# manish-pra/sampling-gpmpc

Measured on AMD Instinct MI355X. Metric: sampled trajectory-steps/sec (Ns*H per wall second), higher is better.
Workload: dtype f64; 1 GPU; BASELINE configs[1]: params_pendulum1D_samples, sequential re-conditioned rollout (mode R, value+gradient labels T=3), Ns=1024 per GPU, H=30; Ns_per_gpu=1024, H=30, Ns_total=1024, device=AMD Radeon Graphics (gfx950:sramecc+:xnack-), cus=256

## Files before the change

### sampling_gpmpc_amd/csrc/rollout_one.hip

```cpp
#include "gpmpc_host.hpp"
#include "rollout_plan.hpp"

#include <type_traits>
#include <utility>

namespace gpmpc {

#include "rollout_one_gen.inc"
#include "rollout_one_steps_gen.inc"

__device__ long long g_one_phase_cycles[16];
__device__ double g_one_dbg[64 * 64];

#ifdef GPMPC_PHASE_TIMERS
#define OPH_DECL long long oph_[10] = {0, 0, 0, 0, 0, 0, 0, 0, 0, 0}; long long opht_ = __builtin_readcyclecounter()
#define OPH(i) do { const long long n_ = __builtin_readcyclecounter(); oph_[i] += n_ - opht_; opht_ = n_; } while (0)
#define OPH_T(i) OPH(i)
#define OPH_STORE do { if (blockIdx.x == 0 && threadIdx.x == 0) { for (int i_ = 0; i_ < 8; ++i_) g_one_phase_cycles[i_] = oph_[i_]; g_one_phase_cycles[10] = oph_[8]; g_one_phase_cycles[11] = oph_[9]; } } while (0)
#elif defined(GPMPC_ONE_PHASE_MARKS)
#define OPH_DECL
#define OPH(i) asm volatile("; one_phase_end " #i)
#define OPH_T(i)
#define OPH_STORE
#else
// ... 207 lines not shown
    if (rk < 0) return OV_OLD;
    if (rk > ri) return OV_ZERO;
    return ri == 0 ? OV_C00 : (ri == 1 ? OV_C10 + rk : OV_C20 + rk);
}
constexpr int one_new_inv(int i) { return (i >= 0 && i < 3) ? OV_CI0 + i : OV_KEEP; }
template <int I0, int BT>
struct OnePatReach {
    static constexpr int at(int kq, int bm, int jq) {
        return (bm == BT && jq < I0 - 1 && kq >= I0) ? one_new_entry(4 + jq - I0, kq - I0) : OV_KEEP;
    }
};
template <int LO>
struct OnePatDiag {
    static constexpr int at(int kq, int bm, int jq) {
        const int ri = 4 * bm + jq - LO;
        return (ri >= 0 && ri < 3) ? one_new_entry(ri, 4 * bm + kq - LO) : OV_KEEP;
    }
};
template <int LO>
struct OnePatInvRow {
    static constexpr int at(int kq, int bm, int) { return one_new_inv(4 * bm + kq - LO); }
};
template <int LO>
struct OnePatInvCol {
    static constexpr int at(int, int bm, int jq) { return one_new_inv(4 * bm + jq - LO); }
};

struct OneCholPair {
    double d0[2], y0[2], r0[2];
};
#ifdef GPMPC_ONE_NO_REST_FENCES
#define GPMPC_ONE_FENCE()
#else
#define GPMPC_ONE_FENCE() __builtin_amdgcn_sched_barrier(0)
#endif
#define GPMPC_ONE_LVL(stmt, third)                              \
    _Pragma("unroll") for (int m_ = 0; m_ < 2; ++m_) { stmt; }  \
    third;                                                      \
    GPMPC_ONE_FENCE()
__device__ __forceinline__ void one_chol_pivot1(double a00, double b00, OneCholPair& p) {
    double h[2], t[2], e[2];
    p.d0[0] = a00, p.d0[1] = b00;
    __builtin_amdgcn_sched_barrier(0);
    GPMPC_ROW2L(p.y0[m_] = __builtin_amdgcn_rsq(p.d0[m_]); h[m_] = 0.5 * p.d0[m_]);
    GPMPC_ROW2L(t[m_] = h[m_] * p.y0[m_]);
    GPMPC_ROW2L(e[m_] = fma(-t[m_], p.y0[m_], 0.5));
    GPMPC_ROW2L(p.y0[m_] = fma(p.y0[m_], e[m_], p.y0[m_]));
    GPMPC_ROW2L(p.r0[m_] = p.d0[m_] * p.y0[m_]);
}
__device__ __forceinline__ void one_chol_rest(const double (&A)[3][3], const double (&B)[3][3], const OneCholPair& p, double x,
                                              const OneExpConsts& k, double (&LA)[3][3], double (&LB)[3][3], double (&invA)[3],
                                              double (&invB)[3], bool& okA, bool& okB, double& ex) {
    double s10[2] = {A[1][0], B[1][0]}, s20[2] = {A[2][0], B[2][0]}, s21[2] = {A[2][1], B[2][1]};
    double s11[2] = {A[1][1], B[1][1]}, s22[2] = {A[2][2], B[2][2]};
    double d1[2], d2[2], y1[2], y2[2], h[2], t[2], e[2], l10[2], l20[2], l21[2], n21[2], p2[2], r1[2], r2[2];
    double n, r, rr, a0, a1, a2, a4;
    int ni;
    GPMPC_ONE_FENCE();
    GPMPC_ONE_LVL(l10[m_] = s10[m_] * p.y0[m_]; l20[m_] = s20[m_] * p.y0[m_], n = x * k.log2e);
    GPMPC_ONE_LVL(d1[m_] = fma(-l10[m_], l10[m_], s11[m_]); n21[m_] = fma(-l20[m_], l10[m_], s21[m_]), n = rint(n));
    GPMPC_ONE_LVL(y1[m_] = __builtin_amdgcn_rsq(d1[m_]); h[m_] = 0.5 * d1[m_]; p2[m_] = fma(-l20[m_], l20[m_], s22[m_]),
                  r = fma(n, k.nln2h, x));
    GPMPC_ONE_LVL(t[m_] = h[m_] * y1[m_], r = fma(n, k.nln2l, r); ni = (int)n);
    GPMPC_ONE_LVL(e[m_] = fma(-t[m_], y1[m_], 0.5), rr = r * r; a0 = 1.0 + r; a1 = fma(k.c3, r, k.c2));
    GPMPC_ONE_LVL(y1[m_] = fma(y1[m_], e[m_], y1[m_]), a0 = fma(a1, rr, a0); a4 = fma(k.c9, r, k.c8); a1 = fma(k.c11, r, k.c10));
    GPMPC_ONE_LVL(l21[m_] = n21[m_] * y1[m_]; r1[m_] = d1[m_] * y1[m_], a4 = fma(a1, rr, a4); a2 = fma(k.c5, r, k.c4));
    GPMPC_ONE_LVL(d2[m_] = fma(-l21[m_], l21[m_], p2[m_]), a1 = fma(k.c7, r, k.c6));
    GPMPC_ONE_LVL(y2[m_] = __builtin_amdgcn_rsq(d2[m_]); h[m_] = 0.5 * d2[m_], a2 = fma(a1, rr, a2); rr = rr * rr);
    GPMPC_ONE_LVL(t[m_] = h[m_] * y2[m_], a2 = fma(a4, rr, a2));
    GPMPC_ONE_LVL(e[m_] = fma(-t[m_], y2[m_], 0.5), a0 = fma(a2, rr, a0));
    GPMPC_ONE_LVL(y2[m_] = fma(y2[m_], e[m_], y2[m_]), ex = ldexp(a0, ni));
    GPMPC_ONE_LVL(r2[m_] = d2[m_] * y2[m_], (void)0);
    asm volatile("" ::"v"(p.r0[0]), "v"(r1[0]), "v"(r2[0]), "v"(p.r0[1]), "v"(r1[1]), "v"(r2[1]));
    okA = (p.d0[0] > 0.0) && (d1[0] > 0.0) && (d2[0] > 0.0);
    okB = (p.d0[1] > 0.0) && (d1[1] > 0.0) && (d2[1] > 0.0);
    LA[0][0] = p.r0[0], LA[1][0] = l10[0], LA[2][0] = l20[0], LA[1][1] = r1[0], LA[2][1] = l21[0], LA[2][2] = r2[0];
    LB[0][0] = p.r0[1], LB[1][0] = l10[1], LB[2][0] = l20[1], LB[1][1] = r1[1], LB[2][1] = l21[1], LB[2][2] = r2[1];
    LA[0][1] = LA[0][2] = LA[1][2] = 0.0;
    LB[0][1] = LB[0][2] = LB[1][2] = 0.0;
    invA[0] = p.y0[0], invA[1] = y1[0], invA[2] = y2[0];
    invB[0] = p.y0[1], invB[1] = y1[1], invB[2] = y2[1];
}

typedef const __attribute__((address_space(4))) RolloutArgs* OneArgsPtr;
typedef __attribute__((address_space(3))) double* OneLdsRow;
__device__ __forceinline__ OneArgsPtr one_cold_args(OneArgsPtr p) {
    asm volatile("" : "+s"(p));
    return p;
}
__device__ __forceinline__ long one_cold_sample(int s) {
    asm volatile("" : "+s"(s));
    return s;
}

__device__ __forceinline__ bool one_wanted(double* p) {
    asm volatile("" : "+s"(p));
    return p != nullptr;
}
struct OneLds {
    static constexpr int VR = 0;
    static constexpr int HS = ((4 * kOneNKT * kOneRS + 1) & ~1);
    static constexpr int TOTAL = HS + 96 * kOneRS;
};

constexpr int one_epoch_of(int t) { return (kOneNKT + ((3 * t) >> 2)) >> 2; }
template <int N0, int ENV, bool LEAN, bool STEPS>
__device__ __forceinline__ void rollout_one_body(const RolloutArgs& a) {
    static_assert(ENV == GPMPC_ENV_PENDULUM1D && N0 == 4, "instantiated for the pendulum1D 4 x 9 grid");
    constexpr int D = 2, T = 3, N1 = 9, NR = N0 * N1, NX = 2;
    constexpr int NKT = kOneNKT;
    constexpr int KFIRST = NKT >> 2, KLAST = (NKT + kOneNTR - 1) >> 2;
    static_assert(4 * NKT == NR && N0 + N1 <= 16, "panel map generated for N_r = 36");
    extern __shared__ __attribute__((aligned(16))) double smem[];
#ifdef GPMPC_PHASE_TIMERS
    const long long opk0_ = __builtin_readcyclecounter();
#endif

    const GpParams& gp = a.gp;
    const OneArgsPtr ak0 = (OneArgsPtr)__builtin_amdgcn_kernarg_segment_ptr();
    const int s32 = blockIdx.x;
    const int lane = threadIdx.x;
    const int kq = lane >> 4, bm = (lane >> 2) & 3, jq = lane & 3;
    const long s = blockIdx.x;
    const int H = a.H;
    double* VRb = smem + OneLds::VR;
    double* HSb = smem + OneLds::HS;

    const double il0 = gp.inv_l2[0][0], il1 = gp.inv_l2[0][1], os = gp.os[0];
    const int lr = (lane < NR) ? lane : 0, ga = lr / N1, gc = lr - ga * N1;
    double qa[N0], qb[N1];
#pragma unroll
    for (int j = 0; j < N0; ++j) qa[j] = plan_grid_Qa(a.plan, gp, 0)[j * N0 + ga];
#pragma unroll
    for (int j = 0; j < N1; ++j) qb[j] = plan_grid_Qb(a.plan, gp, 0)[j * N1 + gc];
    double dsc_ld = plan_grid_dsc(a.plan, gp, 0)[lr], w_ld = plan_grid_w(a.plan, gp, 0)[lr];
    const bool g_ax0 = lane < N0;
    const int g_pt = g_ax0 ? lane * N1 : ((lane < N0 + N1) ? lane - N0 : 0);
    const bool g_axis = lane < N0 + N1, g_sel0 = g_ax0 || !g_axis;
    double g_x = a.X_r[g_pt * D + (g_ax0 ? 0 : 1)];
    const double il0_lane = g_axis ? (g_ax0 ? il0 : il1) : il0, il1_lane = g_axis ? 0.0 : il1;
    const int bp_addr = (lane & 15) << 2;
    constexpr int kPt0 = N0 + N1;
    const int jpt = lane - kPt0;
    const double Inat = (kq == jq) ? 1.0 : 0.0;
    const double MK[4] = {(bm == 0) ? 1.0 : 0.0, (bm == 1) ? 1.0 : 0.0, (bm == 2) ? 1.0 : 0.0, (bm == 3) ? 1.0 : 0.0};
    const int vr_rd = (4 * bm + kq) * kOneRS + jq;
    const int hs_rd = (4 * (bm - NKT) + kq) * kOneRS + jq;
    unsigned hs_wr = (unsigned)(size_t)(OneLdsRow)(HSb + 3 * jpt * kOneRS), vr_wr = (unsigned)(size_t)(OneLdsRow)(VRb + lane * kOneRS);
    asm volatile("" : "+v"(hs_wr), "+v"(vr_wr));
    const int rA = 4 * bm + jq;

    double x[NX];
#pragma unroll
    for (int d = 0; d < NX; ++d) x[d] = a.x0[(a.x0_per_sample ? s * NX : 0) + d];
    double xq[NX] = {0.0, 0.0};
    double zq[T], uq;
    const int lz = (lane < H) ? lane : 0;
#pragma unroll
    for (int c = 0; c < T; ++c) zq[c] = a.z[(long)lz * a.z_step_stride + s * T + c];
    uq = a.u_ff[lz];
    double ud = Inat, drow = 1.0, dcol = 1.0, ud1 = Inat, drow1 = 1.0, dcol1 = 1.0;
    int info_acc = 0;
    double s_min = __builtin_inf();
    int n_h = 0, t = 0;

    double* const Y_s = a.Y ? a.Y + s * H * T : nullptr;
    double* const Xi_s = a.Xi ? a.Xi + s * H * D : nullptr;
    OneExpConsts ek;
    ek.load();
    OnePanels P;
    one_init(P, Inat);
    asm volatile("" : "+v"(qa[0]), "+v"(qa[1]), "+v"(qa[2]), "+v"(qa[3]), "+v"(qb[0]), "+v"(qb[1]), "+v"(qb[2]), "+v"(qb[3]), "+v"(qb[4]),
                 "+v"(qb[5]), "+v"(qb[6]), "+v"(qb[7]), "+v"(qb[8]), "+v"(dsc_ld), "+v"(w_ld), "+v"(g_x), "+v"(x[0]), "+v"(x[1]),
                 "+v"(zq[0]), "+v"(zq[1]), "+v"(zq[2]), "+v"(uq));
    const double dsc = (lane < NR) ? dsc_ld : 0.0, w_lane = (lane < NR) ? w_ld : 0.0;
#pragma unroll
    for (int c = 0; c < T; ++c) zq[c] = (lane < H) ? zq[c] : 0.0;
    uq = (lane < H) ? uq : 0.0;
    double xh[D] = {g_axis ? g_x : 0.0, 0.0}, yt[T] = {0.0, 0.0, 0.0};
    OPH_DECL;
#ifdef GPMPC_PHASE_TIMERS
    if (blockIdx.x == 0 && threadIdx.x == 0) g_one_phase_cycles[8] = opht_ - opk0_;
#endif

    auto ent_a = [&](int tn, bool store, const double (&xs)[NX], double& un) -> double {
        double xi[D];
        {
            const double uf = readlane_f64(uq, tn);
            if (a.env.use_feedback) {
                double acc = 0.0;
#pragma unroll
                for (int j = 0; j < NX; ++j) acc += (a.env.x_goal[j] - xs[j]) * a.env.K[0][j];
                un = -acc + uf;
            } else {
                un = uf;
            }
            xi[0] = xs[0];
            xi[1] = un;
        }
#pragma unroll
        for (int d = 0; d < NX; ++d) xq[d] = (lane == tn) ? xs[d] : xq[d];
        if (!LEAN && lane == 0 && one_wanted(Xi_s) && store) {
#pragma unroll
            for (int d = 0; d < D; ++d) Xi_s[tn * D + d] = xi[d];
        }
        const double d0 = xh[0] - (g_sel0 ? xi[0] : xi[1]), d1 = xh[1] - xi[1], q0 = d0 * il0_lane, q1 = d1 * il1_lane;
        return -0.5 * (d0 * q0 + d1 * q1);
    };
    auto ent_b = [&](int tn, double ea, double xi0, double xi1, double& kk, double& Rq0, double& Rq1) {
        const double gq = (xh[0] - (g_sel0 ? xi0 : xi1)) * il0_lane;
        kk = (jpt >= 0 && jpt < tn) ? os * ea : 0.0;
        Rq0 = one_bpermute(ea, bp_addr);
        Rq1 = one_bpermute(ea * gq, bp_addr);
    };
    struct OneEntC {
        double vr[T], hs[T][T];
    };
    auto ent_c_vals = [&](bool rows, double kk, double xi0, double xi1, double Rq0, double Rq1, OneEntC& e) {
        const double q0 = (xh[0] - xi0) * il0, q1 = (xh[1] - xi1) * il1;
        {
            double PA0 = 0.0, PA1 = 0.0, PB0 = 0.0, PB1 = 0.0;
            one_axis4(PA0, PA1, Rq0, Rq1, qa);
            one_axis9(PB0, PB1, Rq0, Rq1, qb);
            const double s0 = dsc * PB0;
            e.vr[0] = s0 * PA0;
            e.vr[1] = s0 * PA1;
            e.vr[2] = dsc * PA0 * PB1;
        }
        if (rows) {
            const double kA[T] = {kk, -kk * q0, -kk * q1}, kd[T] = {0.0, kk * il0, kk * il1};
#pragma unroll
            for (int aa = 0; aa < T; ++aa) {
                e.hs[aa][0] = kA[aa];
                e.hs[aa][1] = fma(kA[aa], q0, (aa == 1) ? kd[1] : 0.0);
                e.hs[aa][2] = fma(kA[aa], q1, (aa == 2) ? kd[2] : 0.0);
            }
        }
    };
    constexpr unsigned long long kPtLanes = ((1ull << 32) - 1) << kPt0;
    constexpr unsigned long long kRealLanes = (1ull << NR) - 1;
    static_assert(kPtLanes == 0x00001fffffffe000ull && kRealLanes == 0x0000000fffffffffull, "the EXEC literals of ent_c_put");
    auto ent_c_put = [&](auto nhc, const OneEntC& e) {
        constexpr int nh = decltype(nhc)::value;
        constexpr int i0 = nh & 3, ycol = (i0 + 3) & 3;
        constexpr int cb0 = i0, cb1 = (i0 + 1) & 3, cb2 = (i0 + 2) & 3;
        const unsigned ha = hs_wr, va = vr_wr;
        double vr4[4];
        vr4[cb0] = e.vr[0], vr4[cb1] = e.vr[1], vr4[cb2] = e.vr[2], vr4[ycol] = w_lane;
        if constexpr (nh > 0) {
            double h4[T][4];
#pragma unroll
            for (int aa = 0; aa < T; ++aa)
                h4[aa][cb0] = e.hs[aa][0], h4[aa][cb1] = e.hs[aa][1], h4[aa][cb2] = e.hs[aa][2], h4[aa][ycol] = yt[aa];
            asm volatile("s_mov_b32 exec_lo, 0xffffe000\n\ts_mov_b32 exec_hi, 0x1fff\n\t"
                         "ds_write2_b64 %[ha], %[a0], %[a1] offset1:1\n\t"
                         "ds_write2_b64 %[ha], %[a2], %[a3] offset0:2 offset1:3\n\t"
                         "ds_write2_b64 %[ha], %[b0], %[b1] offset0:5 offset1:6\n\t"
                         "ds_write2_b64 %[ha], %[b2], %[b3] offset0:7 offset1:8\n\t"
                         "ds_write2_b64 %[ha], %[c0], %[c1] offset0:10 offset1:11\n\t"
                         "ds_write2_b64 %[ha], %[c2], %[c3] offset0:12 offset1:13\n\t"
                         "s_mov_b32 exec_lo, -1\n\ts_mov_b32 exec_hi, 0xf\n\t"
                         "ds_write2_b64 %[va], %[v0], %[v1] offset1:1\n\t"
                         "ds_write2_b64 %[va], %[v2], %[v3] offset0:2 offset1:3\n\t"
                         "s_mov_b64 exec, -1"
                         :
                         : [ha] "v"(ha), [va] "v"(va), [a0] "v"(h4[0][0]), [a1] "v"(h4[0][1]), [a2] "v"(h4[0][2]), [a3] "v"(h4[0][3]),
                           [b0] "v"(h4[1][0]), [b1] "v"(h4[1][1]), [b2] "v"(h4[1][2]), [b3] "v"(h4[1][3]), [c0] "v"(h4[2][0]),
                           [c1] "v"(h4[2][1]), [c2] "v"(h4[2][2]), [c3] "v"(h4[2][3]), [v0] "v"(vr4[0]), [v1] "v"(vr4[1]), [v2] "v"(vr4[2]),
                           [v3] "v"(vr4[3])
                         : "memory");
        } else {
            asm volatile("s_mov_b32 exec_lo, -1\n\ts_mov_b32 exec_hi, 0xf\n\t"
                         "ds_write2_b64 %[va], %[v0], %[v1] offset1:1\n\t"
                         "ds_write2_b64 %[va], %[v2], %[v3] offset0:2 offset1:3\n\t"
                         "s_mov_b64 exec, -1"
                         :
                         : [va] "v"(va), [v0] "v"(vr4[0]), [v1] "v"(vr4[1]), [v2] "v"(vr4[2]), [v3] "v"(vr4[3])
                         : "memory");
        }
    };

    double ucur;
    {
        double kk, Rq0, Rq1;
        const double ea = one_exp_neg(ent_a(0, true, x, ucur), ek);
        ent_b(0, ea, x[0], ucur, kk, Rq0, Rq1);
        OneEntC e;
        ent_c_vals(false, kk, x[0], ucur, Rq0, Rq1, e);
        ent_c_put(std::integral_constant<int, 0>{}, e);
    }
#ifdef GPMPC_PHASE_TIMERS
    opht_ = __builtin_readcyclecounter();
#endif
    OPH_MARK("end prologue");

    auto finish = [&](double xe0, double xe1) __attribute__((always_inline)) {
        const double xe[NX] = {xe0, xe1};
        if (s_min < gp.var_floor) info_acc |= GPMPC_INFO_VAR_CLAMPED;
        {
            const OneArgsPtr ak = one_cold_args(ak0);
            const long se = one_cold_sample(s32);
            double* const X_traj = ak->X_traj;
            if (lane <= H) {
#pragma unroll
                for (int d = 0; d < NX; ++d) X_traj[(se * NX + d) * (H + 1) + lane] = (lane == H) ? xe[d] : xq[d];
            }
            if (lane == 0) ak->info[se] = info_acc;
        }
        OPH_STORE;
#ifdef GPMPC_PHASE_TIMERS
        if (blockIdx.x == 0 && threadIdx.x == 0) g_one_phase_cycles[9] = __builtin_readcyclecounter() - opk0_;
#endif
    };

    auto step = [&](auto Kc, auto TSc, auto&& next) {
        constexpr int K = decltype(Kc)::value;
        constexpr int TS = decltype(TSc)::value;
        constexpr bool ST = TS >= 0;
        static_assert(!ST || (one_epoch_of(TS) == K && TS >= OneEpoch<K>::t_begin && TS < OneEpoch<K>::t_end), "step outside its epoch");
        constexpr int R0 = 4 * K - NKT;
        const int tl = ST ? TS : t, nhl = ST ? T * TS : n_h;
        const int i0 = nhl & 3, ycol = (i0 + 3) & 3, npts = tl;
        const int cb0 = i0, cb1 = (i0 + 1) & 3, cb2 = (i0 + 2) & 3;
        const bool more = (ST && TS >= kOneAppendSteps) ? false : tl + 1 < H;
        if constexpr (ST) OPH_STEP(TS);
        one_sync_lds();
        double Vu[K + 1], RN[K + 1];
        Vu[0] = VRb[vr_rd];
        Vu[1] = VRb[vr_rd + 16 * kOneRS];
        double t8 = VRb[(32 + kq) * kOneRS + jq];
#pragma unroll
        for (int g = KFIRST; g <= K; ++g) RN[g] = HSb[max(hs_rd + 16 * g * kOneRS, 0)];
        asm volatile("" : "+v"(t8), "+v"(RN[K]));
        Vu[2] = (bm == 0) ? t8 : 0.0;
#pragma unroll
        for (int g = 3; g <= K; ++g) Vu[g] = 0.0;
        OPH(0);

        double S0, S1;
        if constexpr (ST) one_solve_t<TS>(P, Vu, RN, MK, S0, S1, ud, drow, dcol, Inat);
        else one_solve<K>(P, Vu, RN, MK, n_h, S0, S1, ud, drow, dcol, Inat);
        ODBG(0, Vu[0]);
        ODBG(1, Vu[1]);
        ODBG(2, Vu[2]);
        if constexpr (K >= 3) ODBG(3, Vu[3]);
        ODBG(5, RN[2]);
        OPH(2);

        double mu[T], S[T][T], zt[T];
        const double Stot = one_block_sum(S0 + S1);
        ODBG(6, Stot);
        const int cb[T] = {cb0, cb1, cb2};
        auto extract = [&](auto bc) {
            constexpr int bq = decltype(bc)::value;
#pragma unroll
            for (int c = 0; c <= bq; ++c) {
                const double kss = (bq == c) ? ((bq == 0) ? os : ((bq == 1) ? os * il0 : os * il1)) : 0.0;
                const double val = kss - readlane_f64(Stot, 16 * cb[bq] + cb[c]);
                S[bq][c] = val;
                S[c][bq] = val;
            }
        };
        auto var = [&](int bq) { return fmax(S[bq][bq], gp.var_floor); };
        auto fetch = [&](auto bc) {
            constexpr int bq = decltype(bc)::value;
            mu[bq] = readlane_f64(Stot, 16 * cb[bq] + ycol);
            zt[bq] = readlane_f64(zq[bq], tl);
        };
        extract(std::integral_constant<int, 0>{});
        fetch(std::integral_constant<int, 0>{});
        OPH(3);
        OneCholPair ch;
        one_chol_pivot1(S[0][0] + gp.noise[0], S[0][0], ch);
        double y0s;
        {
            double acc = 0.0;
            acc = fma(ch.r0[1], zt[0], acc);
            y0s = acc + mu[0];
        }
        double x0n, un, kk, Rq0, Rq1;
        x0n = x[0] + x[1] * a.env.dt;
        {
            const bool mine = jpt == npts;
            xh[0] = mine ? x[0] : xh[0];
            xh[1] = mine ? ucur : xh[1];
        }
        double earg;
        {
            const double xs[NX] = {x0n, x[1] + y0s};
            earg = ent_a(tl + 1, more, xs, un);
        }
        extract(std::integral_constant<int, 1>{});
        extract(std::integral_constant<int, 2>{});
        one_min3(s_min, S[0][0], S[1][1], S[2][2]);
        bool all_zero = false;
        if (!LEAN && a.var_zero_thr >= 0.0) all_zero = (var(0) <= a.var_zero_thr) && (var(1) <= a.var_zero_thr) && (var(2) <= a.var_zero_thr);
        double Rt[T][T], C[T][T], cinv[T];
        bool c_ok, r_ok;
        {
            double Sn[T][T], rinv[T], ea;
#pragma unroll
            for (int bq = 0; bq < T; ++bq)
#pragma unroll
                for (int c = 0; c < T; ++c) Sn[bq][c] = S[bq][c] + ((bq == c) ? gp.noise[bq] : 0.0);
            one_chol_rest(Sn, S, ch, earg, ek, C, Rt, cinv, rinv, c_ok, r_ok, ea);
            ent_b(tl + 1, ea, x0n, un, kk, Rq0, Rq1);
        }
        fetch(std::integral_constant<int, 1>{});
        fetch(std::integral_constant<int, 2>{});
        double y[T];
        bool clip;
        auto draw = [&]() {
            clip = false;
#pragma unroll
            for (int bq = 0; bq < T; ++bq) {
                double acc = 0.0;
#pragma unroll
                for (int c = 0; c <= bq; ++c) acc = fma(Rt[bq][c], zt[c], acc);
                const double yb = acc + mu[bq];
                const double dlt = yb - mu[bq];
                clip = clip || (dlt * dlt > a.beta * a.beta * S[bq][bq]);
                y[bq] = yb;
            }
        };
        auto cold = [&]() __attribute__((always_inline)) {
            OPH_MARK("cold begin");
            if (all_zero) {
#pragma unroll
                for (int bq = 0; bq < T; ++bq) y[bq] = mu[bq];
                clip = false;
            }
            if (clip) {
#pragma unroll
                for (int bq = 0; bq < T; ++bq) {
                    const double dlt = y[bq] - mu[bq];
                    if (dlt * dlt > a.beta * a.beta * var(bq)) {
                        const double sd = a.beta * sqrt(var(bq));
                        y[bq] = fmin(fmax(y[bq], mu[bq] - sd), mu[bq] + sd);
                    }
                }
            }
            if (y[0] != y0s) {
                const double xs[NX] = {x0n, x[1] + y[0]};
                const double ea = one_exp_neg(ent_a(tl + 1, more, xs, un), ek);
                ent_b(tl + 1, ea, x0n, un, kk, Rq0, Rq1);
            }
            OPH_MARK("cold end");
        };
        if constexpr (!ST) {
            if (__builtin_expect(!r_ok, 0)) info_acc |= root_small_fast_retry<T>(S, one_cold_args(ak0)->gp.jitter, Rt);
            draw();
            if (__builtin_expect(clip || all_zero || !r_ok, 0)) cold();
        } else {
            draw();
            if (__builtin_expect(clip || all_zero || !r_ok || !more, 0)) {
                if (!r_ok) {
                    info_acc |= root_small_fast_retry<T>(S, one_cold_args(ak0)->gp.jitter, Rt);
                    draw();
                }
                if (clip || all_zero || !r_ok) cold();
                if (!more) {
                    finish(x0n, x[1] + y[0]);
                    asm volatile("s_endpgm" : : : "memory");
                }
            }
        }
        if (!LEAN && lane == 0 && one_wanted(Y_s)) {
#pragma unroll
            for (int bq = 0; bq < T; ++bq) Y_s[tl * T + bq] = y[bq];
        }
        OPH(4);

        auto handover = [&]() __attribute__((always_inline)) {
            x[1] = x[1] + y[0];
            x[0] = x0n;
            ucur = un;
        };
        if constexpr (!ST || TS < kOneAppendSteps)
        if (ST || more) {
            if (!c_ok) info_acc |= GPMPC_INFO_TRAIN_CHOL_FAIL;
            {
                const bool mine = jpt == npts;
#pragma unroll
                for (int bq = 0; bq < T; ++bq) yt[bq] = mine ? y[bq] : yt[bq];
            }
            OneEntC ec;
            ent_c_vals(true, kk, x0n, un, Rq0, Rq1, ec);
            const double sv[OV_COUNT] = {0.0, C[0][0], C[1][0], C[1][1], C[2][0], C[2][1], C[2][2], cinv[0], cinv[1], cinv[2], Vu[K]};
            auto inverse_tiles = [&](double U, double dr, double dcl) -> double {
                const double M = Inat - dr * U;
                const double Mt = one_mfma_zero(M, Inat);
                const double M2 = one_mfma_zero(Mt, M);
                const double Pq = one_mfma_zero(Inat + Mt, Inat + M2);
                return Pq * dcl;
            };
            constexpr bool INV_IN_SOLVE = K >= kOneSolveInvK;
            constexpr int TB = OneEpoch<K>::t_begin, TE = OneEpoch<K>::t_end < kOneAppendSteps ? OneEpoch<K>::t_end : kOneAppendSteps;
            auto block = [&](auto tc) {
                constexpr int TT = decltype(tc)::value, NH = T * TT;
                constexpr int i0 = NH & 3;
                constexpr int tn = NH >> 2;
                constexpr int bt = (NKT + tn) & 3;
                constexpr int lo = NH - 4 * R0;
                static_assert(((NKT + tn) >> 2) == K && lo == 4 * bt + i0 && tn >= 0 && tn < kOneNTR, "step outside its epoch");
#ifdef GPMPC_ONE_DEBUG
                if (nhl != NH) g_one_dbg[63 * 64 + lane] = (double)(nhl - NH);
#endif
                ent_c_put(std::integral_constant<int, NH + T>{}, ec);
                OPH(1);
                one_hset_row_at<tn, NH>(Vu);
                if constexpr (i0 >= 2 && tn + 1 < kOneNTR) {
                    double Vm[K + 2];
#pragma unroll
                    for (int gg = 0; gg <= K; ++gg) Vm[gg] = Vu[gg];
                    Vm[K + 1] = 0.0;
                    Vm[K] = one_apply<OnePatReach<i0, bt>>(Vu[K], sv);
                    one_hset_row_at<tn + 1, NH>(Vm);
                }
                OPH(5);
                ud = one_apply<OnePatDiag<lo>>(ud, sv);
                drow = one_apply<OnePatInvRow<lo>>(drow, sv);
                dcol = one_apply<OnePatInvCol<lo>>(dcol, sv);
                OPH_T(9);
                if constexpr (K < KLAST && lo + 3 > 16) {
                    ud1 = one_apply<OnePatDiag<lo - 16>>(ud1, sv);
                    drow1 = one_apply<OnePatInvRow<lo - 16>>(drow1, sv);
                    dcol1 = one_apply<OnePatInvCol<lo - 16>>(dcol1, sv);
                    const double G1 = inverse_tiles(ud1, drow1, dcol1);
                    one_hset_gd<K + 1>(G1);
                }
                if constexpr (INV_IN_SOLVE && TT == OneEpoch<K>::t_end - 1) one_hset_gd<K>(inverse_tiles(ud, drow, dcol));
            };
            if constexpr (!ST) one_pick_row<TB, TE>(t, block);
            else if constexpr (TS < kOneAppendSteps) block(TSc);
            one_for<(R0 > 0 ? R0 : 0), (R0 + 5 < kOneNTR ? R0 + 5 : kOneNTR)>([&](auto rc) { one_touch_row<decltype(rc)::value>(P); });
            if constexpr (K < KLAST) one_touch_gd<K + 1>(P);
            OPH_T(8);
            if constexpr (INV_IN_SOLVE) {
                one_touch_gd<K>(P);
            } else {
                const double Gt = inverse_tiles(ud, drow, dcol);
                ODBG(8, ud);
                ODBG(9, Gt);
                one_put_gd<K>(P, Gt);
            }
            if constexpr (!ST) n_h += T;
        }
        OPH(6);
        handover();
        if constexpr (!ST) t += 1;
        OPH(7);
        if constexpr (ST) next();
    };

    if constexpr (!STEPS) {
        one_for<KFIRST, KLAST + 1>([&](auto Kc) {
            constexpr int K = decltype(Kc)::value;
#pragma unroll 1
            while (t < H && t < OneEpoch<K>::t_end) step(Kc, std::integral_constant<int, -1>{}, [] {});
            ud = ud1, drow = drow1, dcol = dcol1;
            ud1 = Inat, drow1 = 1.0, dcol1 = 1.0;
        });
    } else {
        auto run = [&](auto& self, auto tc) __attribute__((always_inline)) -> void {
            constexpr int TS = decltype(tc)::value, K = one_epoch_of(TS);
            step(std::integral_constant<int, K>{}, tc, [&]() __attribute__((always_inline)) {
                if constexpr (TS < kOneAppendSteps) {
                    if constexpr (TS + 1 == OneEpoch<K>::t_end) {
                        ud = ud1, drow = drow1, dcol = dcol1;
                        ud1 = Inat, drow1 = 1.0, dcol1 = 1.0;
                    }
                    self(self, std::integral_constant<int, TS + 1>{});
                }
            });
        };
        run(run, std::integral_constant<int, 0>{});
    }

    if constexpr (!STEPS) finish(x[0], x[1]);
}

template <int N0, int ENV, bool LEAN>
__global__ __launch_bounds__(64, 1) void rollout_one_kernel(const RolloutArgs a) {
    rollout_one_body<N0, ENV, LEAN, false>(a);
}
template <int N0, int ENV>
__global__ __launch_bounds__(64, 1) void rollout_one_steps_kernel(const RolloutArgs a) {
// ... 45 lines not shown
```

### sampling_gpmpc_amd/csrc/rollout_one_gen.inc

```
__device__ __forceinline__ void one_pchain1(double& c0, double& c1, double a0, double b0) {
    asm volatile("s_nop 1\n\t"
        "v_mfma_f64_4x4x4_4b_f64 %0, %2, %3, %0\n\t"
        "s_nop 5"
        : "+v"(c0), "+v"(c1)
        : "v"(a0), "v"(b0));
}
__device__ __forceinline__ void one_pchain2(double& c0, double& c1, double a0, double a1, double b0, double b1) {
    asm volatile("s_nop 1\n\t"
        "v_mfma_f64_4x4x4_4b_f64 %0, %2, %3, %0\n\t"
        "s_nop 1\n\t"
        "v_mfma_f64_4x4x4_4b_f64 %1, %4, %5, %1\n\t"
        "s_nop 5"
        : "+v"(c0), "+v"(c1)
        : "v"(a0), "v"(b0), "v"(a1), "v"(b1));
}
__device__ __forceinline__ void one_pchain3(double& c0, double& c1, double a0, double a1, double a2, double b0, double b1, double b2) {
    asm volatile("s_nop 1\n\t"
        "v_mfma_f64_4x4x4_4b_f64 %0, %2, %3, %0\n\t"
        "s_nop 1\n\t"
        "v_mfma_f64_4x4x4_4b_f64 %1, %4, %5, %1\n\t"
        "s_nop 1\n\t"
        "v_mfma_f64_4x4x4_4b_f64 %0, %6, %7, %0\n\t"
        "s_nop 5"
        : "+v"(c0), "+v"(c1)
// ... 4796 lines not shown
template <int R>
__device__ __forceinline__ void one_put_gd(OnePanels& P, double v) {
    if constexpr (R == 2) one_put_gd_2(P, v);
    else if constexpr (R == 3) one_put_gd_3(P, v);
    else if constexpr (R == 4) one_put_gd_4(P, v);
    else if constexpr (R == 5) one_put_gd_5(P, v);
    else if constexpr (R == 6) one_put_gd_6(P, v);
    else if constexpr (R == 7) one_put_gd_7(P, v);
}
template <int R>
__device__ __forceinline__ void one_hset_gd(double v) {
    if constexpr (R == 2) one_hset_gd_2(v);
    else if constexpr (R == 3) one_hset_gd_3(v);
    else if constexpr (R == 4) one_hset_gd_4(v);
    else if constexpr (R == 5) one_hset_gd_5(v);
    else if constexpr (R == 6) one_hset_gd_6(v);
    else if constexpr (R == 7) one_hset_gd_7(v);
}
template <int R>
__device__ __forceinline__ void one_touch_gd(OnePanels& P) {
    if constexpr (R == 2) one_touch_gd_2(P);
    else if constexpr (R == 3) one_touch_gd_3(P);
    else if constexpr (R == 4) one_touch_gd_4(P);
    else if constexpr (R == 5) one_touch_gd_5(P);
    else if constexpr (R == 6) one_touch_gd_6(P);
    else if constexpr (R == 7) one_touch_gd_7(P);
}
constexpr int kOneAppendSteps = 29;
template <int K> struct OneEpoch;
template <> struct OneEpoch<2> { static constexpr int t_begin = 0, t_end = 4; };
template <> struct OneEpoch<3> { static constexpr int t_begin = 4, t_end = 10; };
template <> struct OneEpoch<4> { static constexpr int t_begin = 10, t_end = 15; };
template <> struct OneEpoch<5> { static constexpr int t_begin = 15, t_end = 20; };
template <> struct OneEpoch<6> { static constexpr int t_begin = 20, t_end = 26; };
template <> struct OneEpoch<7> { static constexpr int t_begin = 26, t_end = 30; };
template <int R, int NH> struct OneRowMask;
template <> struct OneRowMask<0, 0> { static constexpr unsigned long long base = 0x7777777777777777ull, last = 0x0007000700070007ull; };
template <> struct OneRowMask<0, 3> { static constexpr unsigned long long base = 0x8888888888888888ull, last = 0x0008000800080008ull; };
template <> struct OneRowMask<1, 3> { static constexpr unsigned long long base = 0x3333333333333333ull, last = 0x0033003300330033ull; };
template <> struct OneRowMask<1, 6> { static constexpr unsigned long long base = 0xccccccccccccccccull, last = 0x00cc00cc00cc00ccull; };
template <> struct OneRowMask<2, 6> { static constexpr unsigned long long base = 0x1111111111111111ull, last = 0x0111011101110111ull; };
template <> struct OneRowMask<2, 9> { static constexpr unsigned long long base = 0xeeeeeeeeeeeeeeeeull, last = 0x0eee0eee0eee0eeeull; };
template <> struct OneRowMask<3, 12> { static constexpr unsigned long long base = 0x7777777777777777ull, last = 0x0000000000000000ull; };
template <> struct OneRowMask<3, 15> { static constexpr unsigned long long base = 0x8888888888888888ull, last = 0x0000000000000000ull; };
template <> struct OneRowMask<4, 15> { static constexpr unsigned long long base = 0x3333333333333333ull, last = 0x0003000300030003ull; };
template <> struct OneRowMask<4, 18> { static constexpr unsigned long long base = 0xccccccccccccccccull, last = 0x000c000c000c000cull; };
template <> struct OneRowMask<5, 18> { static constexpr unsigned long long base = 0x1111111111111111ull, last = 0x0011001100110011ull; };
template <> struct OneRowMask<5, 21> { static constexpr unsigned long long base = 0xeeeeeeeeeeeeeeeeull, last = 0x00ee00ee00ee00eeull; };
template <> struct OneRowMask<6, 24> { static constexpr unsigned long long base = 0x7777777777777777ull, last = 0x0777077707770777ull; };
template <> struct OneRowMask<6, 27> { static constexpr unsigned long long base = 0x8888888888888888ull, last = 0x0888088808880888ull; };
template <> struct OneRowMask<7, 27> { static constexpr unsigned long long base = 0x3333333333333333ull, last = 0x0000000000000000ull; };
template <> struct OneRowMask<7, 30> { static constexpr unsigned long long base = 0xccccccccccccccccull, last = 0x0000000000000000ull; };
template <> struct OneRowMask<8, 30> { static constexpr unsigned long long base = 0x1111111111111111ull, last = 0x0001000100010001ull; };
template <> struct OneRowMask<8, 33> { static constexpr unsigned long long base = 0xeeeeeeeeeeeeeeeeull, last = 0x000e000e000e000eull; };
template <> struct OneRowMask<9, 36> { static constexpr unsigned long long base = 0x7777777777777777ull, last = 0x0077007700770077ull; };
template <> struct OneRowMask<9, 39> { static constexpr unsigned long long base = 0x8888888888888888ull, last = 0x0088008800880088ull; };
template <> struct OneRowMask<10, 39> { static constexpr unsigned long long base = 0x3333333333333333ull, last = 0x0333033303330333ull; };
template <> struct OneRowMask<10, 42> { static constexpr unsigned long long base = 0xccccccccccccccccull, last = 0x0ccc0ccc0ccc0cccull; };
template <> struct OneRowMask<11, 42> { static constexpr unsigned long long base = 0x1111111111111111ull, last = 0x0000000000000000ull; };
template <> struct OneRowMask<11, 45> { static constexpr unsigned long long base = 0xeeeeeeeeeeeeeeeeull, last = 0x0000000000000000ull; };
template <> struct OneRowMask<12, 48> { static constexpr unsigned long long base = 0x7777777777777777ull, last = 0x0007000700070007ull; };
template <> struct OneRowMask<12, 51> { static constexpr unsigned long long base = 0x8888888888888888ull, last = 0x0008000800080008ull; };
template <> struct OneRowMask<13, 51> { static constexpr unsigned long long base = 0x3333333333333333ull, last = 0x0033003300330033ull; };
template <> struct OneRowMask<13, 54> { static constexpr unsigned long long base = 0xccccccccccccccccull, last = 0x00cc00cc00cc00ccull; };
template <> struct OneRowMask<14, 54> { static constexpr unsigned long long base = 0x1111111111111111ull, last = 0x0111011101110111ull; };
template <> struct OneRowMask<14, 57> { static constexpr unsigned long long base = 0xeeeeeeeeeeeeeeeeull, last = 0x0eee0eee0eee0eeeull; };
template <> struct OneRowMask<15, 60> { static constexpr unsigned long long base = 0x7777777777777777ull, last = 0x0000000000000000ull; };
template <> struct OneRowMask<15, 63> { static constexpr unsigned long long base = 0x8888888888888888ull, last = 0x0000000000000000ull; };
template <> struct OneRowMask<16, 63> { static constexpr unsigned long long base = 0x3333333333333333ull, last = 0x0003000300030003ull; };
template <> struct OneRowMask<16, 66> { static constexpr unsigned long long base = 0xccccccccccccccccull, last = 0x000c000c000c000cull; };
template <> struct OneRowMask<17, 66> { static constexpr unsigned long long base = 0x1111111111111111ull, last = 0x0011001100110011ull; };
template <> struct OneRowMask<17, 69> { static constexpr unsigned long long base = 0xeeeeeeeeeeeeeeeeull, last = 0x00ee00ee00ee00eeull; };
template <> struct OneRowMask<18, 72> { static constexpr unsigned long long base = 0x7777777777777777ull, last = 0x0777077707770777ull; };
template <> struct OneRowMask<18, 75> { static constexpr unsigned long long base = 0x8888888888888888ull, last = 0x0888088808880888ull; };
template <> struct OneRowMask<19, 75> { static constexpr unsigned long long base = 0x3333333333333333ull, last = 0x0000000000000000ull; };
template <> struct OneRowMask<19, 78> { static constexpr unsigned long long base = 0xccccccccccccccccull, last = 0x0000000000000000ull; };
template <> struct OneRowMask<20, 78> { static constexpr unsigned long long base = 0x1111111111111111ull, last = 0x0001000100010001ull; };
template <> struct OneRowMask<20, 81> { static constexpr unsigned long long base = 0xeeeeeeeeeeeeeeeeull, last = 0x000e000e000e000eull; };
template <> struct OneRowMask<21, 84> { static constexpr unsigned long long base = 0x7777777777777777ull, last = 0x0077007700770077ull; };
template <int R, int NH>
__device__ __forceinline__ void one_hset_row_at(const double* V) {
    one_hset_row<R>(OneRowMask<R, NH>::base, OneRowMask<R, NH>::last, V);
}
```

Baseline: 537.8 million trajectory-steps/s.

## Specialize unrolled steps with per-lane compile-time masks for Cholesky and lane updates

After: 551.0 million trajectory-steps/s (median of 6 runs). 2.5% higher.

```diff
diff --git a/sampling_gpmpc_amd/csrc/rollout_one.hip b/sampling_gpmpc_amd/csrc/rollout_one.hip
--- a/sampling_gpmpc_amd/csrc/rollout_one.hip
+++ b/sampling_gpmpc_amd/csrc/rollout_one.hip
@@ -313,6 +313,75 @@
     invB[0] = p.y0[1], invB[1] = y1[1], invB[2] = y2[1];
 }
 
+template <unsigned long long M>
+__device__ __forceinline__ void one_root_in(double& s11, double& s22, double& y0, double n1, double n2, double y0a) {
+    asm("s_mov_b32 exec_lo, %[lo]\n\ts_mov_b32 exec_hi, %[hi]\n\t"
+        "v_add_f64 %[s11], %[s11], %[n1]\n\tv_add_f64 %[s22], %[s22], %[n2]\n\tv_mov_b64 %[y0], %[y0a]\n\t"
+        "s_mov_b64 exec, -1"
+        : [s11] "+v"(s11), [s22] "+v"(s22), [y0] "+v"(y0)
+        : [n1] "s"(n1), [n2] "s"(n2), [y0a] "v"(y0a), [lo] "n"((int)(unsigned)(M & 0xffffffffull)), [hi] "n"((int)(unsigned)(M >> 32)));
+}
+#define GPMPC_ONE_LVL1(stmt, third) \
+    stmt;                           \
+    third;                          \
+    GPMPC_ONE_FENCE()
+__device__ __forceinline__ void one_chol_rest1(double s10, double s20, double s21, double s11, double s22, double y0, double x,
+                                               const OneExpConsts& k, double& l10, double& l20, double& l21, double& r1, double& r2,
+                                               double& y1, double& y2, double& d2, double& ex) {
+    double d1, h, t, e, n21, p2;
+    double n, r, rr, a0, a1, a2, a4;
+    int ni;
+    GPMPC_ONE_FENCE();
+    GPMPC_ONE_LVL1(l10 = s10 * y0; l20 = s20 * y0, n = x * k.log2e);
+    GPMPC_ONE_LVL1(d1 = fma(-l10, l10, s11); n21 = fma(-l20, l10, s21), n = rint(n));
+    GPMPC_ONE_LVL1(y1 = __builtin_amdgcn_rsq(d1); h = 0.5 * d1; p2 = fma(-l20, l20, s22), r = fma(n, k.nln2h, x));
+    GPMPC_ONE_LVL1(t = h * y1, r = fma(n, k.nln2l, r); ni = (int)n);
+    GPMPC_ONE_LVL1(e = fma(-t, y1, 0.5), rr = r * r; a0 = 1.0 + r; a1 = fma(k.c3, r, k.c2));
+    GPMPC_ONE_LVL1(y1 = fma(y1, e, y1), a0 = fma(a1, rr, a0); a4 = fma(k.c9, r, k.c8); a1 = fma(k.c11, r, k.c10));
+    GPMPC_ONE_LVL1(l21 = n21 * y1; r1 = d1 * y1, a4 = fma(a1, rr, a4); a2 = fma(k.c5, r, k.c4));
+    GPMPC_ONE_LVL1(d2 = fma(-l21, l21, p2), a1 = fma(k.c7, r, k.c6));
+    GPMPC_ONE_LVL1(y2 = __builtin_amdgcn_rsq(d2); h = 0.5 * d2, a2 = fma(a1, rr, a2); rr = rr * rr);
+    GPMPC_ONE_LVL1(t = h * y2, a2 = fma(a4, rr, a2));
+    GPMPC_ONE_LVL1(e = fma(-t, y2, 0.5), a0 = fma(a2, rr, a0));
+    GPMPC_ONE_LVL1(y2 = fma(y2, e, y2), ex = ldexp(a0, ni));
+    GPMPC_ONE_LVL1(r2 = d2 * y2, (void)0);
+    asm volatile("" ::"v"(r1), "v"(r2));
+}
+template <int L>
+__device__ __forceinline__ void one_lane_put(double& x0, double& x1, double v0, double v1) {
+    asm("s_bfm_b64 exec, 1, %[l]\n\tv_mov_b64 %[x0], %[v0]\n\tv_mov_b64 %[x1], %[v1]\n\ts_mov_b64 exec, -1"
+        : [x0] "+v"(x0), [x1] "+v"(x1)
+        : [v0] "v"(v0), [v1] "v"(v1), [l] "n"(L));
+}
+template <int L>
+__device__ __forceinline__ void one_lane_put(double& x0, double& x1, double& x2, double v0, double v1, double v2) {
+    asm("s_bfm_b64 exec, 1, %[l]\n\tv_mov_b64 %[x0], %[v0]\n\tv_mov_b64 %[x1], %[v1]\n\tv_mov_b64 %[x2], %[v2]\n\ts_mov_b64 exec, -1"
+        : [x0] "+v"(x0), [x1] "+v"(x1), [x2] "+v"(x2)
+        : [v0] "v"(v0), [v1] "v"(v1), [v2] "v"(v2), [l] "n"(L));
+}
+template <int L>
+__device__ __forceinline__ void one_lane_put_s(double& x0, double& x1, double& x2, double v0, double v1, double v2) {
+    asm("s_bfm_b64 exec, 1, %[l]\n\tv_mov_b64 %[x0], %[v0]\n\tv_mov_b64 %[x1], %[v1]\n\tv_mov_b64 %[x2], %[v2]\n\ts_mov_b64 exec, -1"
+        : [x0] "+v"(x0), [x1] "+v"(x1), [x2] "+v"(x2)
+        : [v0] "v"(v0), [v1] "s"(v1), [v2] "s"(v2), [l] "n"(L));
+}
+template <class Pat>
+constexpr unsigned long long one_pat_root_lanes() {
+    unsigned long long m = 0;
+    for (int id = OV_C00; id <= OV_CI2; ++id) m |= OnePatIds<Pat>::mask(id);
+    return m;
+}
+template <int TS>
+constexpr unsigned long long one_root_lanes() {
+    if constexpr (TS >= 0) return OneRootLanes<TS>::value;
+    else return 0;
+}
+template <int TS>
+constexpr int one_root_draw_lane() {
+    if constexpr (TS >= 0) return OneRootLanes<TS>::draw;
+    else return 0;
+}
+
 typedef const __attribute__((address_space(4))) RolloutArgs* OneArgsPtr;
 typedef __attribute__((address_space(3))) double* OneLdsRow;
 __device__ __forceinline__ OneArgsPtr one_cold_args(OneArgsPtr p) {
@@ -380,6 +449,12 @@
     unsigned hs_wr = (unsigned)(size_t)(OneLdsRow)(HSb + 3 * jpt * kOneRS), vr_wr = (unsigned)(size_t)(OneLdsRow)(VRb + lane * kOneRS);
     asm volatile("" : "+v"(hs_wr), "+v"(vr_wr));
     const int rA = 4 * bm + jq;
+    constexpr int kVrZero = kOneRS - 1;
+    int t8_rd = (bm == 0) ? (32 + kq) * kOneRS + jq : kVrZero;
+    if constexpr (STEPS) {
+        asm volatile("" : "+v"(t8_rd));
+        if (lane == 0) VRb[kVrZero] = 0.0;
+    }
 
     double x[NX];
 #pragma unroll
@@ -414,7 +489,19 @@
     if (blockIdx.x == 0 && threadIdx.x == 0) g_one_phase_cycles[8] = opht_ - opk0_;
 #endif
 
-    auto ent_a = [&](int tn, bool store, const double (&xs)[NX], double& un) -> double {
+    auto axis_d0 = [&](auto lq, double xi0, double xi1) -> double {
+        if constexpr (decltype(lq)::value >= 0) {
+            double d = xh[0] - xi0;
+            asm("s_bfm_b64 exec, %[w], %[o]\n\tv_add_f64 %[d], %[x], -%[b]\n\ts_mov_b64 exec, -1"
+                : [d] "+v"(d)
+                : [x] "v"(xh[0]), [b] "v"(xi1), [w] "n"(N1), [o] "n"(N0));
+            return d;
+        } else {
+            return xh[0] - (g_sel0 ? xi0 : xi1);
+        }
+    };
+    auto ent_a = [&](auto lq, int tn, bool store, const double (&xs)[NX], double& un) -> double {
+        constexpr int LQ = decltype(lq)::value;
         double xi[D];
         {
             const double uf = readlane_f64(uq, tn);
@@ -429,18 +516,31 @@
             xi[0] = xs[0];
             xi[1] = un;
         }
-#pragma unroll
-        for (int d = 0; d < NX; ++d) xq[d] = (lane == tn) ? xs[d] : xq[d];
+        if constexpr (LQ >= 0) {
+            static_assert(NX == 2, "one statement for the two coordinates");
+            one_lane_put<LQ>(xq[0], xq[1], xs[0], xs[1]);
+        } else {
+#pragma unroll
+            for (int d = 0; d < NX; ++d) xq[d] = (lane == tn) ? xs[d] : xq[d];
+        }
         if (!LEAN && lane == 0 && one_wanted(Xi_s) && store) {
 #pragma unroll
             for (int d = 0; d < D; ++d) Xi_s[tn * D + d] = xi[d];
         }
-        const double d0 = xh[0] - (g_sel0 ? xi[0] : xi[1]), d1 = xh[1] - xi[1], q0 = d0 * il0_lane, q1 = d1 * il1_lane;
+        const double d0 = axis_d0(lq, xi[0], xi[1]), d1 = xh[1] - xi[1], q0 = d0 * il0_lane, q1 = d1 * il1_lane;
         return -0.5 * (d0 * q0 + d1 * q1);
     };
-    auto ent_b = [&](int tn, double ea, double xi0, double xi1, double& kk, double& Rq0, double& Rq1) {
-        const double gq = (xh[0] - (g_sel0 ? xi0 : xi1)) * il0_lane;
-        kk = (jpt >= 0 && jpt < tn) ? os * ea : 0.0;
+    auto ent_b = [&](auto lq, int tn, double ea, double xi0, double xi1, double& kk, double& Rq0, double& Rq1) {
+        constexpr int LQ = decltype(lq)::value;
+        const double gq = axis_d0(lq, xi0, xi1) * il0_lane;
+        if constexpr (LQ > 0) {
+            kk = 0.0;
+            asm("s_bfm_b64 exec, %[w], %[o]\n\tv_mul_f64 %[k], %[os], %[ea]\n\ts_mov_b64 exec, -1"
+                : [k] "+v"(kk)
+                : [os] "s"(os), [ea] "v"(ea), [w] "n"(LQ), [o] "n"(kPt0));
+        } else {
+            kk = (jpt >= 0 && jpt < tn) ? os * ea : 0.0;
+        }
         Rq0 = one_bpermute(ea, bp_addr);
         Rq1 = one_bpermute(ea * gq, bp_addr);
     };
@@ -514,8 +614,8 @@
     double ucur;
     {
         double kk, Rq0, Rq1;
-        const double ea = one_exp_neg(ent_a(0, true, x, ucur), ek);
-        ent_b(0, ea, x[0], ucur, kk, Rq0, Rq1);
+        const double ea = one_exp_neg(ent_a(std::integral_constant<int, -1>{}, 0, true, x, ucur), ek);
+        ent_b(std::integral_constant<int, -1>{}, 0, ea, x[0], ucur, kk, Rq0, Rq1);
         OneEntC e;
         ent_c_vals(false, kk, x[0], ucur, Rq0, Rq1, e);
         ent_c_put(std::integral_constant<int, 0>{}, e);
@@ -559,11 +659,12 @@
         double Vu[K + 1], RN[K + 1];
         Vu[0] = VRb[vr_rd];
         Vu[1] = VRb[vr_rd + 16 * kOneRS];
-        double t8 = VRb[(32 + kq) * kOneRS + jq];
+        double t8 = VRb[ST ? t8_rd : (32 + kq) * kOneRS + jq];
 #pragma unroll
         for (int g = KFIRST; g <= K; ++g) RN[g] = HSb[max(hs_rd + 16 * g * kOneRS, 0)];
         asm volatile("" : "+v"(t8), "+v"(RN[K]));
-        Vu[2] = (bm == 0) ? t8 : 0.0;
+        if constexpr (ST) Vu[2] = t8;
+        else Vu[2] = (bm == 0) ? t8 : 0.0;
 #pragma unroll
         for (int g = 3; g <= K; ++g) Vu[g] = 0.0;
         OPH(0);
@@ -611,7 +712,9 @@
         }
         double x0n, un, kk, Rq0, Rq1;
         x0n = x[0] + x[1] * a.env.dt;
-        {
+        if constexpr (ST) {
+            one_lane_put<kPt0 + (ST ? TS : 0)>(xh[0], xh[1], x[0], ucur);
+        } else {
             const bool mine = jpt == npts;
             xh[0] = mine ? x[0] : xh[0];
             xh[1] = mine ? ucur : xh[1];
@@ -619,7 +722,7 @@
         double earg;
         {
             const double xs[NX] = {x0n, x[1] + y0s};
-            earg = ent_a(tl + 1, more, xs, un);
+            earg = ent_a(std::integral_constant<int, ST ? TS + 1 : -1>{}, tl + 1, more, xs, un);
         }
         extract(std::integral_constant<int, 1>{});
         extract(std::integral_constant<int, 2>{});
@@ -628,14 +731,31 @@
         if (!LEAN && a.var_zero_thr >= 0.0) all_zero = (var(0) <= a.var_zero_thr) && (var(1) <= a.var_zero_thr) && (var(2) <= a.var_zero_thr);
         double Rt[T][T], C[T][T], cinv[T];
         bool c_ok, r_ok;
-        {
+        unsigned long long okb = 0, clipm = 0;
+        constexpr unsigned long long AT = one_root_lanes<TS>();
+        constexpr int RL = one_root_draw_lane<TS>(), PL = kPt0 + (ST ? TS : 0);
+        static_assert(!ST || (!((AT >> RL) & 1) && (RL == PL || ((AT >> PL) & 1))), "the draw's lane factors S");
+        if constexpr (ST) {
+            double s11 = S[1][1], s22 = S[2][2], y0m = ch.y0[1], l10, l20, l21, r1, r2, y1, y2, d2, ea;
+            if constexpr (AT != 0) one_root_in<AT>(s11, s22, y0m, gp.noise[1], gp.noise[2], ch.y0[0]);
+            one_chol_rest1(S[1][0], S[2][0], S[2][1], s11, s22, y0m, earg, ek, l10, l20, l21, r1, r2, y1, y2, d2, ea);
+            okb = __builtin_amdgcn_ballot_w64(d2 > 0.0);
+            c_ok = (okb & AT) == AT;
+            r_ok = (okb & ~AT) == ~AT;
+            C[0][0] = ch.r0[0], C[1][0] = l10, C[2][0] = l20, C[1][1] = r1, C[2][1] = l21, C[2][2] = r2;
+            Rt[0][0] = ch.r0[1], Rt[1][0] = l10, Rt[2][0] = l20, Rt[1][1] = r1, Rt[2][1] = l21, Rt[2][2] = r2;
+            C[0][1] = C[0][2] = C[1][2] = 0.0;
+            Rt[0][1] = Rt[0][2] = Rt[1][2] = 0.0;
+            cinv[0] = ch.y0[0], cinv[1] = y1, cinv[2] = y2;
+            ent_b(std::integral_constant<int, ST ? TS + 1 : -1>{}, tl + 1, ea, x0n, un, kk, Rq0, Rq1);
+        } else {
             double Sn[T][T], rinv[T], ea;
 #pragma unroll
             for (int bq = 0; bq < T; ++bq)
 #pragma unroll
                 for (int c = 0; c < T; ++c) Sn[bq][c] = S[bq][c] + ((bq == c) ? gp.noise[bq] : 0.0);
             one_chol_rest(Sn, S, ch, earg, ek, C, Rt, cinv, rinv, c_ok, r_ok, ea);
-            ent_b(tl + 1, ea, x0n, un, kk, Rq0, Rq1);
+            ent_b(std::integral_constant<int, -1>{}, tl + 1, ea, x0n, un, kk, Rq0, Rq1);
         }
         fetch(std::integral_constant<int, 1>{});
         fetch(std::integral_constant<int, 2>{});
@@ -643,6 +763,7 @@
         bool clip;
         auto draw = [&]() {
             clip = false;
+            clipm = 0;
 #pragma unroll
             for (int bq = 0; bq < T; ++bq) {
                 double acc = 0.0;
@@ -650,9 +771,12 @@
                 for (int c = 0; c <= bq; ++c) acc = fma(Rt[bq][c], zt[c], acc);
                 const double yb = acc + mu[bq];
                 const double dlt = yb - mu[bq];
-                clip = clip || (dlt * dlt > a.beta * a.beta * S[bq][bq]);
+                const bool cl = dlt * dlt > a.beta * a.beta * S[bq][bq];
+                if constexpr (ST) clipm |= __builtin_amdgcn_ballot_w64(cl);
+                else clip = clip || cl;
                 y[bq] = yb;
             }
+            if constexpr (ST) clip = (clipm & ~AT) != 0;
         };
         auto cold = [&]() __attribute__((always_inline)) {
             OPH_MARK("cold begin");
@@ -673,8 +797,8 @@
             }
             if (y[0] != y0s) {
                 const double xs[NX] = {x0n, x[1] + y[0]};
-                const double ea = one_exp_neg(ent_a(tl + 1, more, xs, un), ek);
-                ent_b(tl + 1, ea, x0n, un, kk, Rq0, Rq1);
+                const double ea = one_exp_neg(ent_a(std::integral_constant<int, -1>{}, tl + 1, more, xs, un), ek);
+                ent_b(std::integral_constant<int, -1>{}, tl + 1, ea, x0n, un, kk, Rq0, Rq1);
             }
             OPH_MARK("cold end");
         };
@@ -684,7 +808,7 @@
             if (__builtin_expect(clip || all_zero || !r_ok, 0)) cold();
         } else {
             draw();
-            if (__builtin_expect(clip || all_zero || !r_ok || !more, 0)) {
+            if (__builtin_expect(((~okb | (clipm & ~AT)) != 0) || all_zero || !more, 0)) {
                 if (!r_ok) {
                     info_acc |= root_small_fast_retry<T>(S, one_cold_args(ak0)->gp.jitter, Rt);
                     draw();
@@ -694,6 +818,8 @@
                     finish(x0n, x[1] + y[0]);
                     asm volatile("s_endpgm" : : : "memory");
                 }
+                if constexpr (TS < kOneAppendSteps)
+                    if (!c_ok) info_acc |= GPMPC_INFO_TRAIN_CHOL_FAIL;
             }
         }
         if (!LEAN && lane == 0 && one_wanted(Y_s)) {
@@ -709,8 +835,13 @@
         };
         if constexpr (!ST || TS < kOneAppendSteps)
         if (ST || more) {
-            if (!c_ok) info_acc |= GPMPC_INFO_TRAIN_CHOL_FAIL;
-            {
+            if constexpr (!ST)
+                if (!c_ok) info_acc |= GPMPC_INFO_TRAIN_CHOL_FAIL;
+            if constexpr (ST && RL == PL) {
+                one_lane_put<PL>(yt[0], yt[1], yt[2], y[0], y[1], y[2]);
+            } else if constexpr (ST) {
+                one_lane_put_s<PL>(yt[0], yt[1], yt[2], y[0], readlane_f64(y[1], RL), readlane_f64(y[2], RL));
+            } else {
                 const bool mine = jpt == npts;
 #pragma unroll
                 for (int bq = 0; bq < T; ++bq) yt[bq] = mine ? y[bq] : yt[bq];
@@ -734,6 +865,14 @@
                 constexpr int bt = (NKT + tn) & 3;
                 constexpr int lo = NH - 4 * R0;
                 static_assert(((NKT + tn) >> 2) == K && lo == 4 * bt + i0 && tn >= 0 && tn < kOneNTR, "step outside its epoch");
+                static_assert(OneRootLanes<TT>::value ==
+                                  (((i0 >= 2 && tn + 1 < kOneNTR) ? one_pat_root_lanes<OnePatReach<i0, bt>>() : 0ull) |
+                                   one_pat_root_lanes<OnePatDiag<lo>>() | one_pat_root_lanes<OnePatInvRow<lo>>() |
+                                   one_pat_root_lanes<OnePatInvCol<lo>>() |
+                                   ((K < KLAST && lo + 3 > 16) ? (one_pat_root_lanes<OnePatDiag<lo - 16>>() | one_pat_root_lanes<OnePatInvRow<lo - 16>>() |
+                                                                one_pat_root_lanes<OnePatInvCol<lo - 16>>())
+                                                             : 0ull)),
+                              "OneRootLanes (tools/gen_rollout_one.py: root_lanes) against the step's patterns");
 #ifdef GPMPC_ONE_DEBUG
                 if (nhl != NH) g_one_dbg[63 * 64 + lane] = (double)(nhl - NH);
 #endif
diff --git a/sampling_gpmpc_amd/csrc/rollout_one_gen.inc b/sampling_gpmpc_amd/csrc/rollout_one_gen.inc
--- a/sampling_gpmpc_amd/csrc/rollout_one_gen.inc
+++ b/sampling_gpmpc_amd/csrc/rollout_one_gen.inc
@@ -4902,3 +4902,34 @@
 __device__ __forceinline__ void one_hset_row_at(const double* V) {
     one_hset_row<R>(OneRowMask<R, NH>::base, OneRowMask<R, NH>::last, V);
 }
+template <int TS> struct OneRootLanes;
+template <> struct OneRootLanes<0> { static constexpr unsigned long long value = 0x007000f000f000f0ull; static constexpr int draw = 13; };
+template <> struct OneRootLanes<1> { static constexpr unsigned long long value = 0x03f003800f800f80ull; static constexpr int draw = 14; };
+template <> struct OneRootLanes<2> { static constexpr unsigned long long value = 0x1f001f001c00fc00ull; static constexpr int draw = 63; };
+template <> struct OneRootLanes<3> { static constexpr unsigned long long value = 0xf000f000f000e000ull; static constexpr int draw = 16; };
+template <> struct OneRootLanes<4> { static constexpr unsigned long long value = 0x0007000f000f000full; static constexpr int draw = 63; };
+template <> struct OneRootLanes<5> { static constexpr unsigned long long value = 0x003f003800f800f8ull; static constexpr int draw = 18; };
+template <> struct OneRootLanes<6> { static constexpr unsigned long long value = 0x01f001f001c00fc0ull; static constexpr int draw = 19; };
+template <> struct OneRootLanes<7> { static constexpr unsigned long long value = 0x0f000f000f000e00ull; static constexpr int draw = 20; };
+template <> struct OneRootLanes<8> { static constexpr unsigned long long value = 0x7000f000f000f000ull; static constexpr int draw = 21; };
+template <> struct OneRootLanes<9> { static constexpr unsigned long long value = 0xf0038003800f800full; static constexpr int draw = 22; };
+template <> struct OneRootLanes<10> { static constexpr unsigned long long value = 0x001f001f001c00fcull; static constexpr int draw = 23; };
+template <> struct OneRootLanes<11> { static constexpr unsigned long long value = 0x00f000f000f000e0ull; static constexpr int draw = 24; };
+template <> struct OneRootLanes<12> { static constexpr unsigned long long value = 0x07000f000f000f00ull; static constexpr int draw = 63; };
+template <> struct OneRootLanes<13> { static constexpr unsigned long long value = 0x3f003800f800f800ull; static constexpr int draw = 26; };
+template <> struct OneRootLanes<14> { static constexpr unsigned long long value = 0xf001f001c001c00full; static constexpr int draw = 27; };
+template <> struct OneRootLanes<15> { static constexpr unsigned long long value = 0x000f000f000f000eull; static constexpr int draw = 28; };
+template <> struct OneRootLanes<16> { static constexpr unsigned long long value = 0x007000f000f000f0ull; static constexpr int draw = 29; };
+template <> struct OneRootLanes<17> { static constexpr unsigned long long value = 0x03f003800f800f80ull; static constexpr int draw = 30; };
+template <> struct OneRootLanes<18> { static constexpr unsigned long long value = 0x1f001f001c00fc00ull; static constexpr int draw = 31; };
+template <> struct OneRootLanes<19> { static constexpr unsigned long long value = 0xf000f000f000e000ull; static constexpr int draw = 32; };
+template <> struct OneRootLanes<20> { static constexpr unsigned long long value = 0x0007000f000f000full; static constexpr int draw = 63; };
+template <> struct OneRootLanes<21> { static constexpr unsigned long long value = 0x003f003800f800f8ull; static constexpr int draw = 34; };
+template <> struct OneRootLanes<22> { static constexpr unsigned long long value = 0x01f001f001c00fc0ull; static constexpr int draw = 35; };
+template <> struct OneRootLanes<23> { static constexpr unsigned long long value = 0x0f000f000f000e00ull; static constexpr int draw = 36; };
+template <> struct OneRootLanes<24> { static constexpr unsigned long long value = 0x7000f000f000f000ull; static constexpr int draw = 37; };
+template <> struct OneRootLanes<25> { static constexpr unsigned long long value = 0xf0038003800f800full; static constexpr int draw = 38; };
+template <> struct OneRootLanes<26> { static constexpr unsigned long long value = 0x001f001f001c00fcull; static constexpr int draw = 39; };
+template <> struct OneRootLanes<27> { static constexpr unsigned long long value = 0x00f000f000f000e0ull; static constexpr int draw = 40; };
+template <> struct OneRootLanes<28> { static constexpr unsigned long long value = 0x07000f000f000f00ull; static constexpr int draw = 63; };
+template <> struct OneRootLanes<29> { static constexpr unsigned long long value = 0x0000000000000000ull; static constexpr int draw = 42; };
```
